# ramkp990/Truth_Recommendation_GNN

Measured on NVIDIA B200. Metric: message-passing edges/s (train step), higher is better.
Workload: dtype f32

## Files before the change

### include/trg_b200.h

```cpp
#ifndef TRG_B200_H
#define TRG_B200_H

#include <stddef.h>
#include <stdint.h>

#ifdef __cplusplus
extern "C" {
#endif

#define TRG_ABI_VERSION 4

enum { TRG_F32 = 0, TRG_BF16 = 1, TRG_F8E4M3 = 2  };
enum {
  TRG_OK = 0,
  TRG_E_ARG = 1,
  TRG_E_WORKSPACE = 2,
  TRG_E_CUDA = 3,
  TRG_E_UNSUPPORTED = 4
};

int trg_abi_version(void);
const char* trg_last_error(void);
int64_t trg_launch_count(void);

size_t trg_csr_workspace_bytes(int64_t n_edges, int64_t n_key);
int trg_csr_build(const int64_t* other, const int64_t* key, int64_t n_edges, int64_t n_key,
                  int32_t* rowptr , int32_t* col , int32_t* eid ,
                  void* workspace, size_t workspace_bytes, void* stream);

size_t trg_select_range_workspace_bytes(int64_t n);
int trg_select_range(const int64_t* key, const int64_t* other, int64_t n, int64_t lo, int64_t hi,
                     int64_t capacity, int64_t pad_key, int64_t pad_other,
                     int64_t* key_out , int64_t* other_out ,
                     int32_t* count_out , void* workspace, size_t workspace_bytes, void* stream);

typedef struct {
  const int32_t* vrowptr;
  const int32_t* vinfo;
  int64_t n_vrows;
  const int32_t* long_rows;
  const int32_t* long_ptr;
  int64_t n_long;
  float* partial;
} trg_long_rows;

int trg_sage_agg_fwd(const int32_t* rowptr, const int32_t* col, const void* x_src,
                     int64_t n_dst, int32_t feat, int dtype,
                     void* mean_out , float* inv_deg_out ,
                     const trg_long_rows* long_rows , void* stream);

int trg_sage_agg_bwd(const int32_t* rowptr_t, const int32_t* col_t, const float* inv_deg,
                     const void* g_mean, int64_t n_src, int32_t feat, int dtype,
                     void* g_src_out , int out_dtype, int accumulate,
                     const void* relu_of, const trg_long_rows* long_rows ,
                     void* stream);

int trg_gather_wsum(const int32_t* rowptr, const int32_t* col, const int32_t* eid,
                    const float* coef, const float* scale, const void* x,
                    int64_t n_rows, int32_t feat, int dtype, void* out, int out_dtype, int accumulate,
                    const void* relu_of, const trg_long_rows* long_rows , void* stream);

int trg_rows_finish(const void* in, int in_dtype, const float* row_scale, const void* add,
                    const void* relu_of, int64_t n_rows, int32_t feat, int dtype, void* out, void* stream);

int trg_peer_reduce_rows(const void* const* parts, int32_t n_peers, int64_t row0, int in_dtype,
                         const float* row_scale, const void* add, const void* relu_of, int64_t n_rows,
                         int32_t feat, int dtype, void* out, int32_t ctas_per_sm, void* stream);

size_t trg_edge_bce_workspace_bytes(int64_t n_users);
int trg_edge_bce_fwd(const int32_t* rowptr_u, const int32_t* col_p, const int32_t* eid,
                     const int64_t* neg_p, const void* u, const void* p,
                     int64_t n_users, int64_t n_edges, int32_t hidden, int dtype,
                     const float* wbar , float* loss_out,
                     float* c_pos, float* c_neg, void* g_u,
                     void* workspace, size_t workspace_bytes, void* stream);

int trg_edge_anchor_loss(const int32_t* rowptr, const int32_t* col, const int32_t* eid,
                         const void* anchor, const void* gathered, int64_t n_rows,
                         int64_t n_edges_scale, int32_t hidden, int dtype, int label,
                         const float* wbar, float* loss_out, float* coef_out, void* g_anchor,
                         int accumulate, int relu_gate, void* workspace, size_t workspace_bytes,
                         void* stream);

typedef struct {
  const void* a;
  const void* w;
  int32_t k;
  float alpha;
} trg_proj_term;
size_t trg_sage_proj_workspace_bytes(int32_t k_total, int32_t hidden, int dtype);
int trg_sage_proj_fwd(const trg_proj_term* terms , int32_t n_terms,
                      const float* bias ,
                      int64_t n_rows, int32_t hidden, int dtype, int relu,
                      void* out ,
                      void* workspace, size_t workspace_bytes, void* stream);

typedef struct {
  const void* w;
  int32_t k;
  float alpha;
  const float* row_scale;
  void* d_a;
} trg_proj_bwd_term;
int trg_sage_proj_bwd_input(const void* dz, const trg_proj_bwd_term* terms , int32_t n_terms,
                            int64_t n_rows, int32_t hidden, int dtype,
                            void* workspace, size_t workspace_bytes, void* stream);

typedef struct {
  const void* a;
  int32_t k;
  float alpha;
  void* d_w;
} trg_proj_dw_term;
size_t trg_sage_proj_dw_workspace_bytes(void);
int trg_sage_proj_bwd_weight(const void* dz, const trg_proj_dw_term* terms , int32_t n_terms,
                             float* d_bias ,
                             int64_t n_rows, int32_t hidden, int dtype,
                             void* workspace, size_t workspace_bytes, void* stream);

size_t trg_score_topk_workspace_bytes(int64_t n_query, int64_t n_cat, int32_t hidden, int32_t k);
int trg_score_topk(const void* q , const void* cat ,
                   int64_t n_query, int64_t n_cat, int32_t hidden, int dtype, int32_t k,
                   int64_t id_offset, float* vals_out , int64_t* ids_out ,
                   void* workspace, size_t workspace_bytes, void* stream);
int trg_score_topk_excluding(const void* q , const void* cat ,
                             int64_t n_query, int64_t n_cat, int32_t hidden, int dtype, int32_t k,
                             int64_t id_offset, const int32_t* excl_rowptr ,
                             const int32_t* excl_ids , const int64_t* query_rows ,
                             float* vals_out , int64_t* ids_out ,
                             void* workspace, size_t workspace_bytes, void* stream);
int trg_topk_merge(const float* vals_in , const int64_t* ids_in,
                   int64_t n_query, int32_t n_lists, int32_t k_in, int32_t k_out,
                   float* vals_out, int64_t* ids_out, void* stream);

size_t trg_rescore_topk_workspace_bytes(int64_t n_query, int32_t n_cand);
int trg_rescore_topk(const void* q , const void* table , int64_t n_query, int64_t n_table,
                     int32_t hidden, int dtype, const int64_t* cand_ids , int32_t n_cand,
                     int64_t id_offset, int32_t k, float* vals_out ,
                     int64_t* ids_out , void* workspace, size_t workspace_bytes, void* stream);

#ifdef __cplusplus
}
#endif
#endif
```

### truth_recommendation_gnn_b200/_lib.py

```python
from __future__ import annotations

import ctypes
import os

import torch

_HERE = os.path.dirname(os.path.abspath(__file__))
LIB_PATH = os.path.join(_HERE, "lib", "libtrg_b200.so")

TRG_F32, TRG_BF16, TRG_F8E4M3 = 0, 1, 2
ABI_VERSION = 4

_vp, _i64, _i32, _sz, _int = ctypes.c_void_p, ctypes.c_int64, ctypes.c_int32, ctypes.c_size_t, ctypes.c_int


class TrgProjTerm(ctypes.Structure):
    _fields_ = [("a", _vp), ("w", _vp), ("k", _i32), ("alpha", ctypes.c_float)]


class TrgLongRows(ctypes.Structure):
    _fields_ = [("vrowptr", _vp), ("vinfo", _vp), ("n_vrows", _i64), ("long_rows", _vp), ("long_ptr", _vp),
                ("n_long", _i64), ("partial", _vp)]


class TrgProjBwdTerm(ctypes.Structure):
    _fields_ = [("w", _vp), ("k", _i32), ("alpha", ctypes.c_float), ("row_scale", _vp), ("d_a", _vp)]


class TrgProjDwTerm(ctypes.Structure):
    _fields_ = [("a", _vp), ("k", _i32), ("alpha", ctypes.c_float), ("d_w", _vp)]


SIGNATURES = {
    "trg_abi_version": (_int, []),
    "trg_last_error": (ctypes.c_char_p, []),
    "trg_launch_count": (_i64, []),
    "trg_csr_workspace_bytes": (_sz, [_i64, _i64]),
    "trg_csr_build": (_int, [_vp, _vp, _i64, _i64, _vp, _vp, _vp, _vp, _sz, _vp]),
    "trg_select_range_workspace_bytes": (_sz, [_i64]),
    "trg_select_range": (_int, [_vp, _vp, _i64, _i64, _i64, _i64, _i64, _i64, _vp, _vp, _vp, _vp, _sz, _vp]),
    "trg_sage_agg_fwd": (_int, [_vp, _vp, _vp, _i64, _i32, _int, _vp, _vp, ctypes.POINTER(TrgLongRows), _vp]),
    "trg_sage_agg_bwd": (_int, [_vp, _vp, _vp, _vp, _i64, _i32, _int, _vp, _int, _int, _vp,
                                ctypes.POINTER(TrgLongRows), _vp]),
    "trg_gather_wsum": (_int, [_vp, _vp, _vp, _vp, _vp, _vp, _i64, _i32, _int, _vp, _int, _int, _vp,
                               ctypes.POINTER(TrgLongRows), _vp]),
    "trg_rows_finish": (_int, [_vp, _int, _vp, _vp, _vp, _i64, _i32, _int, _vp, _vp]),
    "trg_peer_reduce_rows": (_int, [_vp, _i32, _i64, _int, _vp, _vp, _vp, _i64, _i32, _int, _vp, _i32, _vp]),
    "trg_edge_bce_workspace_bytes": (_sz, [_i64]),
    "trg_edge_bce_fwd": (_int, [_vp, _vp, _vp, _vp, _vp, _vp, _i64, _i64, _i32, _int, _vp, _vp,
                                _vp, _vp, _vp, _vp, _sz, _vp]),
    "trg_edge_anchor_loss": (_int, [_vp, _vp, _vp, _vp, _vp, _i64, _i64, _i32, _int, _int, _vp, _vp, _vp,
                                    _vp, _int, _int, _vp, _sz, _vp]),
    "trg_sage_proj_workspace_bytes": (_sz, [_i32, _i32, _int]),
    "trg_sage_proj_fwd": (_int, [ctypes.POINTER(TrgProjTerm), _i32, _vp, _i64, _i32, _int, _int, _vp,
                                 _vp, _sz, _vp]),
    "trg_sage_proj_bwd_input": (_int, [_vp, ctypes.POINTER(TrgProjBwdTerm), _i32, _i64, _i32, _int,
                                       _vp, _sz, _vp]),
    "trg_sage_proj_dw_workspace_bytes": (_sz, []),
    "trg_sage_proj_bwd_weight": (_int, [_vp, ctypes.POINTER(TrgProjDwTerm), _i32, _vp, _i64, _i32, _int,
                                        _vp, _sz, _vp]),
    "trg_score_topk_workspace_bytes": (_sz, [_i64, _i64, _i32, _i32]),
    "trg_score_topk": (_int, [_vp, _vp, _i64, _i64, _i32, _int, _i32, _i64, _vp, _vp, _vp, _sz, _vp]),
    "trg_score_topk_excluding": (_int, [_vp, _vp, _i64, _i64, _i32, _int, _i32, _i64, _vp, _vp, _vp, _vp, _vp,
                                        _vp, _sz, _vp]),
    "trg_topk_merge": (_int, [_vp, _vp, _i64, _i32, _i32, _i32, _vp, _vp, _vp]),
    "trg_rescore_topk_workspace_bytes": (_sz, [_i64, _i32]),
    "trg_rescore_topk": (_int, [_vp, _vp, _i64, _i64, _i32, _int, _vp, _i32, _i64, _i32, _vp, _vp, _vp, _sz,
                                _vp]),
}

_lib = None


class TrgError(RuntimeError):
    pass


def load():
    global _lib
    if _lib is None:
        if not os.path.exists(LIB_PATH):
            raise TrgError(
                f"{LIB_PATH} is missing: build it with `python -m truth_recommendation_gnn_b200.build` "
                "(nvcc, sm_100a). There is no CPU or PyTorch fallback for the hot path.")
        lib = ctypes.CDLL(LIB_PATH)
        for name, (res, args) in SIGNATURES.items():
            fn = getattr(lib, name)
            fn.restype, fn.argtypes = res, args
        if lib.trg_abi_version() != ABI_VERSION:
            raise TrgError("libtrg_b200.so ABI version mismatch; rebuild")
        _lib = lib
    return _lib


def check(rc: int, what: str):
    if rc != 0:
        raise TrgError(f"{what} failed (rc={rc}): {load().trg_last_error().decode()}")


def ptr(t):
    if t is None:
        return None
    if not t.is_cuda:
        raise TrgError("truth_recommendation_gnn_b200 runs on CUDA (sm_100a) tensors only; got a "
                       f"{t.device} tensor. There is no CPU fallback.")
    if not t.is_contiguous():
        raise TrgError("non-contiguous tensor passed to the C ABI")
    return t.data_ptr()


def stream():
    return torch.cuda.current_stream().cuda_stream


def dtype_code(dt: torch.dtype) -> int:
    if dt == torch.float32:
        return TRG_F32
    if dt == torch.bfloat16:
        return TRG_BF16
    raise TrgError(f"unsupported dtype {dt}: the hot path computes in fp32 or bf16 (fp32 accumulate)")


class Profiler:

    def __init__(self):
        self.enabled = False
        self.records = []

    def reset(self):
        self.records = []

    def summary(self):
        out = {}
        for name, nbytes, s, e in self.records:
            d = out.setdefault(name, dict(calls=0, ms=0.0, bytes=0))
            d["calls"] += 1
            d["ms"] += s.elapsed_time(e)
            d["bytes"] += int(nbytes)
        return out


PROF = Profiler()


def call(name, nbytes, fn, *args):
    if PROF.enabled:
        s, e = torch.cuda.Event(enable_timing=True), torch.cuda.Event(enable_timing=True)
        s.record()
        rc = fn(*args)
        e.record()
        PROF.records.append((name, nbytes, s, e))
    else:
        rc = fn(*args)
    check(rc, name)


def launch_count() -> int:
    return int(load().trg_launch_count())
```

### truth_recommendation_gnn_b200/csrc/csr_build.cu

```cuda
#include <algorithm>
#include <cstdio>

#include "common.cuh"

namespace trg {
namespace {

constexpr int kThreads = 256;
constexpr int kItems = 16;
constexpr int kTile = kThreads * kItems;
constexpr int kWarps = kThreads / 32;
constexpr int kRadix = 256;

template <int NWARPS>
__device__ __forceinline__ int block_exclusive_scan(int v, int* warp_sums, int& total) {
  const int lane = threadIdx.x & 31, w = threadIdx.x >> 5;
  int inc = v;
#pragma unroll
  for (int o = 1; o < 32; o <<= 1) {
    int t = __shfl_up_sync(0xffffffffu, inc, o);
    if (lane >= o) inc += t;
  }
  if (lane == 31) warp_sums[w] = inc;
  __syncthreads();
// ... 122 lines not shown
      __trap();
    }
  }
}

__global__ void __launch_bounds__(kThreads)
    select_scatter(const long long* __restrict__ key, const long long* __restrict__ other, int64_t n, long long lo,
                   long long hi, const int* __restrict__ tile_offsets, const int* __restrict__ count,
                   long long capacity, long long pad_key, long long pad_other, long long* __restrict__ key_out,
                   long long* __restrict__ other_out) {
  __shared__ int wtot[kWarps];
  const int lane = threadIdx.x & 31, w = threadIdx.x >> 5;
  const int64_t wbase = (int64_t)blockIdx.x * kTile + (int64_t)w * (kItems * 32);
  long long kv[kItems];
  unsigned sel[kItems];
  int mine = 0;
#pragma unroll
  for (int r = 0; r < kItems; ++r) {
    const int64_t idx = wbase + r * 32 + lane;
    kv[r] = idx < n ? ldg_stream(key + idx) : lo - 1;
    const bool in = kv[r] >= lo && kv[r] < hi;
    sel[r] = __ballot_sync(0xffffffffu, in);
    mine += __popc(sel[r]);
  }
  if (lane == 0) wtot[w] = mine;
  __syncthreads();
  int run = tile_offsets[blockIdx.x];
  for (int i = 0; i < w; ++i) run += wtot[i];
#pragma unroll
  for (int r = 0; r < kItems; ++r) {
    if ((sel[r] >> lane) & 1u) {
      const int dest = run + __popc(sel[r] & ((1u << lane) - 1u));
      if (dest < capacity) {
        key_out[dest] = kv[r] - lo;
        other_out[dest] = ldg_stream(other + wbase + r * 32 + lane);
      }
    }
    run += __popc(sel[r]);
  }
  const long long cnt = *count;
  for (long long i = cnt + (long long)blockIdx.x * kThreads + threadIdx.x; i < capacity;
       i += (long long)gridDim.x * kThreads) {
    key_out[i] = pad_key;
    other_out[i] = pad_other;
  }
}

__device__ __forceinline__ uint2 ldg_pair(const uint2* p) {
  uint2 r;
  asm volatile("ld.global.nc.L1::no_allocate.v2.u32 {%0,%1}, [%2];" : "=r"(r.x), "=r"(r.y) : "l"(p));
  return r;
}
template <bool FIRST>
__device__ __forceinline__ uint32_t load_key(const void* keys, int64_t idx) {
  if (FIRST) return (uint32_t)ldg_stream(reinterpret_cast<const long long*>(keys) + idx);
  return ldg_pair(reinterpret_cast<const uint2*>(keys) + idx).x;
}

template <bool FIRST>
__global__ void __launch_bounds__(kThreads) radix_hist(const void* __restrict__ keys, int64_t n,
                                                       int shift, int* __restrict__ hist,
                                                       int n_ctas) {
  __shared__ int h[kRadix];
  h[threadIdx.x] = 0;
  __syncthreads();
  const int64_t base = (int64_t)blockIdx.x * kTile;
#pragma unroll
  for (int i = 0; i < kItems; ++i) {
    int64_t idx = base + (int64_t)i * kThreads + threadIdx.x;
    if (idx < n) atomicAdd(&h[(load_key<FIRST>(keys, idx) >> shift) & (kRadix - 1)], 1);
  }
  __syncthreads();
  hist[(int64_t)threadIdx.x * n_ctas + blockIdx.x] = h[threadIdx.x];
}

template <bool FIRST, bool LAST>
__global__ void __launch_bounds__(kThreads)
    radix_scatter(const void* __restrict__ keys_in, int64_t n, int shift, const int* __restrict__ gbase,
                  int n_ctas, uint2* __restrict__ pairs_out, uint32_t* __restrict__ vals_out) {
  __shared__ int wcnt[kWarps][kRadix];
  __shared__ int sbase[kRadix];
  const int lane = threadIdx.x & 31, w = threadIdx.x >> 5;
#pragma unroll
  for (int i = 0; i < kWarps; ++i) wcnt[i][threadIdx.x] = 0;
  const int64_t wbase = (int64_t)blockIdx.x * kTile + (int64_t)w * (kItems * 32);

  uint32_t key[kItems], val[kItems];
#pragma unroll
  for (int r = 0; r < kItems; ++r) {
    int64_t idx = wbase + r * 32 + lane;
    bool valid = idx < n;
    if (FIRST) {
      key[r] = valid ? load_key<true>(keys_in, idx) : 0u;
      val[r] = (uint32_t)idx;
    } else {
      const uint2 kv = valid ? ldg_pair(reinterpret_cast<const uint2*>(keys_in) + idx) : make_uint2(0u, 0u);
      key[r] = kv.x;
      val[r] = kv.y;
    }
  }
  __syncthreads();

  int rank[kItems];
#pragma unroll
  for (int r = 0; r < kItems; ++r) {
    const bool valid = wbase + r * 32 + lane < n;
    const int d = valid ? (int)((key[r] >> shift) & (kRadix - 1)) : kRadix;
    const unsigned peers = __match_any_sync(0xffffffffu, d);
    const int prev = valid ? wcnt[w][d] : 0;
    __syncwarp();
    if (valid && lane == __ffs(peers) - 1) wcnt[w][d] = prev + __popc(peers);
    __syncwarp();
    rank[r] = prev + __popc(peers & ((1u << lane) - 1u));
  }
  __syncthreads();
  {
    int run = 0;
#pragma unroll
    for (int i = 0; i < kWarps; ++i) {
      int t = wcnt[i][threadIdx.x];
      wcnt[i][threadIdx.x] = run;
      run += t;
    }
    sbase[threadIdx.x] = gbase[(int64_t)threadIdx.x * n_ctas + blockIdx.x];
  }
  __syncthreads();
#pragma unroll
  for (int r = 0; r < kItems; ++r) {
    if (wbase + r * 32 + lane < n) {
      const int d = (int)((key[r] >> shift) & (kRadix - 1));
      const int dest = sbase[d] + wcnt[w][d] + rank[r];
      if (LAST)
        vals_out[dest] = val[r];
      else
        pairs_out[dest] = make_uint2(key[r], val[r]);
    }
  }
}

__global__ void __launch_bounds__(kThreads) gather_col(const long long* __restrict__ other,
                                                       const int* __restrict__ eid, int64_t n,
                                                       int* __restrict__ col) {
  int64_t i = (int64_t)blockIdx.x * blockDim.x + threadIdx.x;
  const int64_t stride = (int64_t)gridDim.x * blockDim.x;
  for (; i < n; i += stride) col[i] = (int)other[ldg_stream(eid + i)];
}

int num_passes(int64_t n_key) {
  int bits = 1;
  while (bits < 32 && ((int64_t)1 << bits) < n_key) ++bits;
  return (bits + 7) / 8;
}

struct Workspace {
  uint2* pairs[2];
  uint32_t* vals;
  int *hist, *tile_sums;
  size_t bytes;
};

Workspace carve(void* ws, int64_t e, int64_t n_key) {
  Workspace w;
  const size_t ebytes = align_up((size_t)(e > 0 ? e : 1) * 4, 256);
  const int64_t n_ctas = ceil_div<int64_t>(e > 0 ? e : 1, kTile);
  const size_t hist_bytes = align_up((size_t)kRadix * n_ctas * 4, 256);
  const int64_t scan_len = (int64_t)kRadix * n_ctas > n_key + 1 ? (int64_t)kRadix * n_ctas : n_key + 1;
  const size_t sums_bytes = align_up((size_t)ceil_div<int64_t>(scan_len, kTile) * 4 + 4, 256);
  char* p = reinterpret_cast<char*>(ws);
  w.pairs[0] = (uint2*)p; p += 2 * ebytes;
  w.pairs[1] = (uint2*)p; p += 2 * ebytes;
  w.vals = (uint32_t*)p; p += ebytes;
  w.hist = (int*)p; p += hist_bytes;
  w.tile_sums = (int*)p; p += sums_bytes;
  w.bytes = (size_t)(p - reinterpret_cast<char*>(ws));
  return w;
}

}
}

using namespace trg;

extern "C" size_t trg_csr_workspace_bytes(int64_t n_edges, int64_t n_key) {
  if (n_edges < 0 || n_key < 0) return 0;
  return carve(nullptr, n_edges, n_key).bytes;
}

extern "C" int trg_csr_build(const int64_t* other, const int64_t* key, int64_t e, int64_t n_key,
                             int32_t* rowptr, int32_t* col, int32_t* eid, void* workspace,
                             size_t workspace_bytes, void* stream) {
  cudaStream_t st = reinterpret_cast<cudaStream_t>(stream);
  TRG_CHECK_ARG(e >= 0 && n_key >= 0, "trg_csr_build: negative size");
  TRG_CHECK_ARG(e < ((int64_t)1 << 31) && n_key < ((int64_t)1 << 31) - 1,
                "trg_csr_build: n_edges=%lld / n_key=%lld exceed int32 CSR range", (long long)e,
                (long long)n_key);
  TRG_CHECK_ARG(rowptr != nullptr, "trg_csr_build: rowptr is NULL");
  TRG_CHECK_ARG(e == 0 || (key != nullptr && (col == nullptr || other != nullptr)),
                "trg_csr_build: NULL edge arrays with n_edges > 0");
  TRG_CHECK_ARG(e == 0 || n_key > 0, "trg_csr_build: edges present but n_key == 0");
  Workspace w = carve(workspace, e, n_key);
  if (workspace == nullptr || workspace_bytes < w.bytes) {
    set_error("trg_csr_build: workspace %zu < required %zu", workspace_bytes, w.bytes);
    return TRG_E_WORKSPACE;
  }
  TRG_CUDA(cudaMemsetAsync(rowptr, 0, (size_t)(n_key + 1) * sizeof(int32_t), st));
  if (e == 0) return TRG_OK;

  {
    int grid = (int)std::min<int64_t>(ceil_div<int64_t>(e, kThreads), (int64_t)kNumSMs * 16);
    count_keys<<<grid, kThreads, 0, st>>>((const long long*)key, e, (long long)n_key, rowptr);
    count_launch();
    TRG_LAUNCH_OK();
    int rc = exclusive_scan(rowptr, rowptr, n_key + 1, w.tile_sums, st);
    if (rc) return rc;
  }
  if (col == nullptr && eid == nullptr) return TRG_OK;

  const int passes = num_passes(n_key);
  const int n_ctas = (int)ceil_div<int64_t>(e, kTile);
  const void* kin = key;
  const uint32_t* vin = nullptr;
  for (int p = 0; p < passes; ++p) {
    const bool first = p == 0, last = p == passes - 1;
    const int shift = 8 * p;
    uint2* kout = w.pairs[p & 1];
    uint32_t* vout = eid ? (uint32_t*)eid : w.vals;
    if (first)
      radix_hist<true><<<n_ctas, kThreads, 0, st>>>(kin, e, shift, w.hist, n_ctas);
    else
      radix_hist<false><<<n_ctas, kThreads, 0, st>>>(kin, e, shift, w.hist, n_ctas);
    count_launch();
    TRG_LAUNCH_OK();
    int rc = exclusive_scan(w.hist, w.hist, (int64_t)kRadix * n_ctas, w.tile_sums, st);
    if (rc) return rc;
    if (first && last)
      radix_scatter<true, true><<<n_ctas, kThreads, 0, st>>>(kin, e, shift, w.hist, n_ctas, kout, vout);
    else if (first)
      radix_scatter<true, false><<<n_ctas, kThreads, 0, st>>>(kin, e, shift, w.hist, n_ctas, kout, vout);
    else if (last)
      radix_scatter<false, true><<<n_ctas, kThreads, 0, st>>>(kin, e, shift, w.hist, n_ctas, kout, vout);
    else
      radix_scatter<false, false><<<n_ctas, kThreads, 0, st>>>(kin, e, shift, w.hist, n_ctas, kout, vout);
    count_launch();
    TRG_LAUNCH_OK();
    kin = kout;
    vin = vout;
  }
  if (col != nullptr) {
    int grid = (int)std::min<int64_t>(ceil_div<int64_t>(e, kThreads), (int64_t)kNumSMs * 16);
    gather_col<<<grid, kThreads, 0, st>>>((const long long*)other, (const int*)vin, e, col);
    count_launch();
    TRG_LAUNCH_OK();
  }
  return TRG_OK;
}

extern "C" size_t trg_select_range_workspace_bytes(int64_t n) {
  if (n < 0) return 0;
  return align_up((size_t)(ceil_div<int64_t>(n > 0 ? n : 1, kTile) + 1) * 4, 256);
}

extern "C" int trg_select_range(const int64_t* key, const int64_t* other, int64_t n, int64_t lo, int64_t hi,
                                int64_t capacity, int64_t pad_key, int64_t pad_other, int64_t* key_out,
                                int64_t* other_out, int32_t* count_out, void* workspace, size_t workspace_bytes,
                                void* stream) {
  cudaStream_t st = reinterpret_cast<cudaStream_t>(stream);
  TRG_CHECK_ARG(n >= 0 && capacity >= 0 && lo <= hi, "trg_select_range: bad sizes");
  TRG_CHECK_ARG(n < ((int64_t)1 << 31) && capacity < ((int64_t)1 << 31), "trg_select_range: sizes exceed int32 range");
  TRG_CHECK_ARG(count_out && (capacity == 0 || (key_out && other_out)), "trg_select_range: NULL outputs");
  TRG_CHECK_ARG(n == 0 || (key && other), "trg_select_range: NULL inputs with n > 0");
  if (workspace == nullptr || workspace_bytes < trg_select_range_workspace_bytes(n)) {
    set_error("trg_select_range: workspace %zu < required %zu", workspace_bytes, trg_select_range_workspace_bytes(n));
    return TRG_E_WORKSPACE;
  }
  int* tile_counts = reinterpret_cast<int*>(workspace);
  const int n_tiles = (int)ceil_div<int64_t>(n > 0 ? n : 1, kTile);
  select_count<<<n_tiles, kThreads, 0, st>>>((const long long*)key, n, lo, hi, tile_counts);
  select_offsets<<<1, 1024, 0, st>>>(tile_counts, n_tiles, capacity, count_out);
  select_scatter<<<n_tiles, kThreads, 0, st>>>((const long long*)key, (const long long*)other, n, lo, hi, tile_counts,
                                               count_out, capacity, pad_key, pad_other, (long long*)key_out,
                                               (long long*)other_out);
  count_launch(3);
  TRG_LAUNCH_OK();
  return TRG_OK;
}
```

### truth_recommendation_gnn_b200/functional.py

```python
from __future__ import annotations

import ctypes

import torch

from . import _lib, fp8
from .graph import CSR, RelationGraph, build_csr


def _long_rows_arg(csr: CSR, feat: int, dev, elem_size: int = 4):
    lr = csr.long_rows() if feat * elem_size >= 80 else None
    if lr is None:
        return None, None
    partial = torch.empty(lr.n_slots, feat, dtype=torch.float32, device=dev)
    s = _lib.TrgLongRows(_lib.ptr(lr.vrowptr), _lib.ptr(lr.vinfo), int(lr.vinfo.numel()), _lib.ptr(lr.long_rows),
                         _lib.ptr(lr.long_ptr), int(lr.long_rows.numel()), _lib.ptr(partial))
    return ctypes.byref(s), (s, partial)


def _check_rows(x: torch.Tensor, what: str):
    es = x.element_size()
    if x.dim() != 2 or (x.size(1) * es) % 16 != 0:
        raise _lib.TrgError(f"{what}: rows must be a multiple of 16 bytes (got shape {tuple(x.shape)}, "
                            f"{x.dtype}); pad the feature width (the reference pads to 64, inference.py:401-404)")
# ... 29 lines not shown
        raise _lib.TrgError(f"output dtype {out_dtype} is not supported for a {x.dtype} table")
    return out_dtype


def sage_agg_bwd(csr_t: CSR, inv_deg, g_mean: torch.Tensor, out=None, accumulate=False, relu_of=None,
                 out_dtype=None):
    lib = _lib.load()
    g_mean = g_mean.contiguous()
    _check_rows(g_mean, "sage_agg_bwd")
    out_dtype = _out_dtype(g_mean, out, out_dtype)
    _check_epilogue(out, relu_of, csr_t.n_rows, g_mean, "sage_agg_bwd", out_dtype)
    if out is None:
        out = torch.empty(csr_t.n_rows, g_mean.size(1), dtype=out_dtype, device=g_mean.device)
        accumulate = False
    if csr_t.n_rows:
        rb = g_mean.size(1) * g_mean.element_size()
        ob = g_mean.size(1) * out.element_size()
        nbytes = (csr_t.n_edges * (rb + 4) + 4 * (csr_t.n_rows + 1)
                  + csr_t.n_rows * (ob * (1 + bool(accumulate)) + rb * (relu_of is not None))
                  + (4 * csr_t.n_cols if inv_deg is not None else 0))
        lr, keep = _long_rows_arg(csr_t, g_mean.size(1), g_mean.device, g_mean.element_size())
        _lib.call("trg_sage_agg_bwd", nbytes, lib.trg_sage_agg_bwd,
                  _lib.ptr(csr_t.rowptr), _lib.ptr(csr_t.col), _lib.ptr(inv_deg), _lib.ptr(g_mean),
                  csr_t.n_rows, g_mean.size(1), _lib.dtype_code(g_mean.dtype), _lib.ptr(out),
                  _lib.dtype_code(out_dtype), 1 if accumulate else 0, _lib.ptr(relu_of), lr, _lib.stream())
    return out


class SageAggFn(torch.autograd.Function):

    @staticmethod
    def forward(ctx, x_src, rel: RelationGraph, grad_prescaled: bool = False):
        want_inv = rel.inv_deg is None
        mean, inv_deg = sage_agg_fwd(rel.fwd, x_src, want_inv_deg=want_inv)
        if want_inv:
            rel.inv_deg = inv_deg
        ctx.rel = rel
        ctx.grad_prescaled = grad_prescaled
        return mean

    @staticmethod
    def backward(ctx, g_mean):
        if not ctx.needs_input_grad[0]:
            return None, None, None
        rel = ctx.rel
        return sage_agg_bwd(rel.bwd, None if ctx.grad_prescaled else rel.inv_deg, g_mean), None, None


def sage_mean_aggregate(x_src: torch.Tensor, rel: RelationGraph, grad_prescaled: bool = False) -> torch.Tensor:
    return SageAggFn.apply(x_src, rel, grad_prescaled)


def gather_wsum(csr: CSR, coef, x: torch.Tensor, scale=None, out=None, accumulate=False, relu_of=None,
                out_dtype=None):
    lib = _lib.load()
    x = x.contiguous()
    _check_rows(x, "gather_wsum")
    out_dtype = _out_dtype(x, out, out_dtype)
    _check_epilogue(out, relu_of, csr.n_rows, x, "gather_wsum", out_dtype)
    if out is None:
        out = torch.empty(csr.n_rows, x.size(1), dtype=out_dtype, device=x.device)
        accumulate = False
    if csr.n_rows:
        rb = x.size(1) * x.element_size()
        ob = x.size(1) * out.element_size()
        nbytes = (csr.n_edges * (rb + 12) + 4 * (csr.n_rows + 1)
                  + csr.n_rows * (ob * (1 + bool(accumulate)) + rb * (relu_of is not None)))
        lr, keep = _long_rows_arg(csr, x.size(1), x.device, x.element_size())
        _lib.call("trg_gather_wsum", nbytes, lib.trg_gather_wsum,
                  _lib.ptr(csr.rowptr), _lib.ptr(csr.col), _lib.ptr(csr.eid), _lib.ptr(coef),
                  _lib.ptr(scale), _lib.ptr(x), csr.n_rows, x.size(1), _lib.dtype_code(x.dtype),
                  _lib.ptr(out), _lib.dtype_code(out_dtype), 1 if accumulate else 0, _lib.ptr(relu_of), lr,
                  _lib.stream())
    return out


def rows_finish(x, dtype, row_scale=None, add=None, relu_of=None, out=None):
    lib = _lib.load()
    x = x.contiguous()
    n, feat = x.shape
    if x.dtype != dtype and x.dtype != torch.float32:
        raise _lib.TrgError(f"rows_finish: input must be {dtype} or float32, got {x.dtype}")
    for t, what in ((add, "add"), (relu_of, "relu_of"), (out, "out")):
        if t is not None and (t.shape != x.shape or t.dtype != dtype or not t.is_contiguous()):
            raise _lib.TrgError(f"rows_finish: {what} must be a contiguous [{n}, {feat}] {dtype} tensor")
    if out is None:
        out = torch.empty(n, feat, dtype=dtype, device=x.device)
    _check_rows(out, "rows_finish")
    rs = row_scale.float().contiguous() if row_scale is not None else None
    es = out.element_size()
    nbytes = n * feat * (x.element_size() + es * (1 + (add is not None) + (relu_of is not None)))
    _lib.call("trg_rows_finish", nbytes, lib.trg_rows_finish, _lib.ptr(x), _lib.dtype_code(x.dtype), _lib.ptr(rs),
              _lib.ptr(add), _lib.ptr(relu_of), n, feat, _lib.dtype_code(dtype), _lib.ptr(out), _lib.stream())
    return out


def peer_reduce_rows(parts, row0, n_rows, dtype, row_scale=None, add=None, relu_of=None, ctas_per_sm=0):
    import ctypes
    lib = _lib.load()
    feat = parts[0].size(1)
    for t in parts:
        if t.dtype != parts[0].dtype or t.size(1) != feat or t.size(0) < row0 + n_rows or not t.is_contiguous():
            raise _lib.TrgError("peer_reduce_rows: partial tables must be contiguous, of one dtype and width, and "
                                "hold rows [row0, row0 + n_rows)")
    if parts[0].dtype != dtype and parts[0].dtype != torch.float32:
        raise _lib.TrgError(f"peer_reduce_rows: partial tables must be {dtype} or float32")
    for t, what in ((add, "add"), (relu_of, "relu_of")):
        if t is not None and (tuple(t.shape) != (n_rows, feat) or t.dtype != dtype or not t.is_contiguous()):
            raise _lib.TrgError(f"peer_reduce_rows: {what} must be a contiguous [{n_rows}, {feat}] {dtype} tensor")
    out = torch.empty(n_rows, feat, dtype=dtype, device=parts[0].device)
    _check_rows(out, "peer_reduce_rows")
    rs = row_scale.float().contiguous() if row_scale is not None else None
    ptrs = (ctypes.c_void_p * len(parts))(*[_lib.ptr(t) for t in parts])
    nbytes = n_rows * feat * (len(parts) * parts[0].element_size()
                              + out.element_size() * (1 + (add is not None) + (relu_of is not None)))
    _lib.call("trg_peer_reduce_rows", nbytes, lib.trg_peer_reduce_rows, ptrs, len(parts), row0,
              _lib.dtype_code(parts[0].dtype), _lib.ptr(rs), _lib.ptr(add), _lib.ptr(relu_of), n_rows, feat,
              _lib.dtype_code(dtype), _lib.ptr(out), ctas_per_sm, _lib.stream())
    return out


class LinkStructure:

    def __init__(self, train_edge_index, interaction_type_tensor, num_users, num_posts):
        pos_u, pos_p = train_edge_index[0], train_edge_index[1]
        self.train_edge_index = train_edge_index
        self.num_users, self.num_posts = int(num_users), int(num_posts)
        self.n_edges = int(pos_u.numel())
        self.by_user = build_csr(pos_p, pos_u, self.num_users, self.num_posts)
        self.by_post = build_csr(pos_u, pos_p, self.num_posts, self.num_users, validate=False)
        self._by_post_u = None
        self._user_of_u = None
        if self.n_edges:
            w = interaction_type_tensor[pos_p + num_users].float()
            self.wbar = w.mean().reshape(1).contiguous()
        else:
            self.wbar = torch.full((1,), float("nan"), device=pos_u.device)


    @property
    def by_post_u(self) -> CSR:
        if self._by_post_u is None:
            bu, bp = self.by_user, self.by_post
            inv = torch.empty(self.n_edges, dtype=torch.int32, device=bu.eid.device)
            inv[bu.eid.long()] = torch.arange(self.n_edges, dtype=torch.int32, device=bu.eid.device)
            self._by_post_u = CSR(bp.rowptr, bp.col, inv[bp.eid.long()].contiguous(), bp.n_rows, bp.n_cols, bp._long)
        return self._by_post_u

    @property
    def user_of_u(self) -> torch.Tensor:
        if self._user_of_u is None:
            rp = self.by_user.rowptr.long()
            self._user_of_u = torch.repeat_interleave(
                torch.arange(self.num_users, device=rp.device), rp[1:] - rp[:-1]).contiguous()
        return self._user_of_u


_LINK_CACHE: dict = {}


def link_structure(train_edge_index, interaction_type_tensor, num_users, num_posts) -> LinkStructure:
    key = (train_edge_index.data_ptr(), tuple(train_edge_index.shape), train_edge_index._version,
           interaction_type_tensor.data_ptr(), interaction_type_tensor._version, int(num_users),
           int(num_posts))
    s = _LINK_CACHE.get(key)
    if s is None:
        if len(_LINK_CACHE) > 8:
            _LINK_CACHE.clear()
        s = LinkStructure(train_edge_index, interaction_type_tensor, num_users, num_posts)
        s._keepalive = interaction_type_tensor
        _LINK_CACHE[key] = s
    return s


def edge_bce_fwd(ls: LinkStructure, user_emb, post_emb, neg_p, want_grad: bool):
    lib = _lib.load()
    _check_rows(user_emb, "edge_bce_fwd")
    if user_emb.dtype != post_emb.dtype or user_emb.size(1) != post_emb.size(1):
        raise _lib.TrgError("user and post embeddings must share dtype and width")
    if neg_p.dtype != torch.int64 or neg_p.numel() != ls.n_edges:
        raise _lib.TrgError("neg_p must be int64 with one entry per positive edge (train_gnn.py:272)")
    user_emb, post_emb, neg_p = user_emb.contiguous(), post_emb.contiguous(), neg_p.contiguous()
    dev = user_emb.device
    loss = torch.empty(1, dtype=torch.float32, device=dev)
    c_pos = c_neg = g_u = None
    if want_grad:
        c_pos = torch.empty(ls.n_edges, dtype=torch.float32, device=dev)
        c_neg = torch.empty(ls.n_edges, dtype=torch.float32, device=dev)
        g_u = torch.empty_like(user_emb)
    ws_bytes = int(lib.trg_edge_bce_workspace_bytes(ls.num_users))
    ws = torch.empty(ws_bytes, dtype=torch.uint8, device=dev)
    e = ls.n_edges
    e_scale = int(getattr(ls, "n_edges_scale", e))
    rb = user_emb.size(1) * user_emb.element_size()
    nbytes = e * (2 * rb + 16 + (8 if want_grad else 0)) + ls.num_users * (rb * (2 if want_grad else 1) + 4)
    _lib.call("trg_edge_bce_fwd", nbytes, lib.trg_edge_bce_fwd,
              _lib.ptr(ls.by_user.rowptr), _lib.ptr(ls.by_user.col) if e else None,
              _lib.ptr(ls.by_user.eid) if e else None, _lib.ptr(neg_p) if e else None,
              _lib.ptr(user_emb), _lib.ptr(post_emb), ls.num_users, e_scale, user_emb.size(1),
              _lib.dtype_code(user_emb.dtype), _lib.ptr(ls.wbar), _lib.ptr(loss), _lib.ptr(c_pos),
              _lib.ptr(c_neg), _lib.ptr(g_u), _lib.ptr(ws), ws_bytes, _lib.stream())
    return loss, c_pos, c_neg, g_u


def edge_anchor_loss(csr: CSR, anchor, gathered, n_edges_scale, label, wbar, want_grad, g_anchor=None,
                     relu_gate=False, coef_in_csr_order=False):
    lib = _lib.load()
    anchor, gathered = anchor.contiguous(), gathered.contiguous()
    _check_rows(anchor, "edge_anchor_loss")
    dev = anchor.device
    loss = torch.empty(1, dtype=torch.float32, device=dev)
    coef = None
    accumulate = g_anchor is not None
    if want_grad:
        coef = torch.empty(csr.n_edges, dtype=torch.float32, device=dev)
        if g_anchor is None:
            g_anchor = torch.empty_like(anchor)
    else:
        g_anchor = None
    ws_bytes = int(lib.trg_edge_bce_workspace_bytes(csr.n_rows))
    ws = torch.empty(ws_bytes, dtype=torch.uint8, device=dev)
    e = csr.n_edges
    rb = anchor.size(1) * anchor.element_size()
    nbytes = e * (rb + 12) + csr.n_rows * (rb * (2 if want_grad else 1) + 4)
    _lib.call("trg_edge_anchor_loss", nbytes, lib.trg_edge_anchor_loss,
              _lib.ptr(csr.rowptr), _lib.ptr(csr.col) if e else None,
              _lib.ptr(csr.eid) if (e and not coef_in_csr_order) else None,
              _lib.ptr(anchor), _lib.ptr(gathered), csr.n_rows, int(n_edges_scale), anchor.size(1),
              _lib.dtype_code(anchor.dtype), 1 if label else 0, _lib.ptr(wbar), _lib.ptr(loss), _lib.ptr(coef),
              _lib.ptr(g_anchor), 1 if (accumulate and want_grad) else 0,
              1 if (relu_gate and want_grad) else 0, _lib.ptr(ws), ws_bytes, _lib.stream())
    return loss, coef, g_anchor


class LinkBCEFn(torch.autograd.Function):

    @staticmethod
    def forward(ctx, user_emb, post_emb, neg_p, ls: LinkStructure):
        want = user_emb.requires_grad or post_emb.requires_grad
        if neg_p.dtype != torch.int64 or neg_p.numel() != ls.n_edges:
            raise _lib.TrgError("neg_p must be int64 with one entry per positive edge (train_gnn.py:272)")
        if getattr(ls, "eid_long", None) is None:
            ls.eid_long = ls.by_user.eid.long()
        e_scale = int(getattr(ls, "n_edges_scale", ls.n_edges))
        bu = ls.by_user
        ctx.neg_by_post = None
        if want and ls.n_edges:
            ctx.neg_by_post = build_csr(ls.train_edge_index[0], neg_p, ls.num_posts, ls.num_users, validate=False,
                                        per_step=True)
        col_neg = neg_p.index_select(0, ls.eid_long).int()
        neg_csr = CSR(bu.rowptr, col_neg, bu.eid, bu.n_rows, bu.n_cols)
        l_pos, c_pos, g_u = edge_anchor_loss(bu, user_emb, post_emb, e_scale, 1, ls.wbar, want, None)
        l_neg, c_neg, g_u = edge_anchor_loss(neg_csr, user_emb, post_emb, e_scale, 0, ls.wbar, want, g_u)
        ctx.ls = ls
        ctx.want = want
        if want:
            ctx.save_for_backward(user_emb, neg_p, c_pos, c_neg, g_u)
        return (l_pos + l_neg).reshape(())

    @staticmethod
    def backward(ctx, g):
        user_emb, neg_p, c_pos, c_neg, g_u = ctx.saved_tensors
        ls = ctx.ls
        g = g.reshape(1).float().contiguous()
        g_user = g_post = None
        if ctx.needs_input_grad[0]:
            g_user = g_u * g.to(g_u.dtype)
        if ctx.needs_input_grad[1]:
            g_post = gather_wsum(ls.by_post, c_pos, user_emb, scale=g)
            if ctx.neg_by_post is not None:
                gather_wsum(ctx.neg_by_post, c_neg, user_emb, scale=g, out=g_post, accumulate=True)
        return g_user, g_post, None, None


def link_bce_loss(user_emb, post_emb, train_edge_index, neg_p, interaction_type_tensor, num_users):
    ls = link_structure(train_edge_index, interaction_type_tensor, num_users, post_emb.size(0))
    return LinkBCEFn.apply(user_emb, post_emb, neg_p, ls)


def _proj_bytes(n, ks, hidden, es):
    return n * (sum(ks) + hidden) * es


def sage_proj_fwd(terms, bias, relu: bool):
    lib = _lib.load()
    a0 = terms[0][0]
    n, hidden = a0.size(0), terms[0][1].size(0)
    arr = (_lib.TrgProjTerm * len(terms))()
    keep = []
    for i, (a, w, alpha) in enumerate(terms):
        a, w = a.contiguous(), w.contiguous()
        if a.dtype != a0.dtype or w.dtype != a0.dtype:
            raise _lib.TrgError("projection operands must share one dtype")
        keep += [a, w]
        arr[i].a, arr[i].w, arr[i].k, arr[i].alpha = _lib.ptr(a), _lib.ptr(w), a.size(1), float(alpha)
    out = torch.empty(n, hidden, dtype=a0.dtype, device=a0.device)
    b = bias.float().contiguous() if bias is not None else None
    ktot = sum(t[0].size(1) for t in terms)
    code = _lib.dtype_code(a0.dtype)
    ws_bytes = int(lib.trg_sage_proj_workspace_bytes(ktot, hidden, code))
    ws = torch.empty(ws_bytes, dtype=torch.uint8, device=a0.device)
    _lib.call("trg_sage_proj_fwd", _proj_bytes(n, [t[0].size(1) for t in terms], hidden, a0.element_size()),
              lib.trg_sage_proj_fwd, arr, len(terms), _lib.ptr(b), n, hidden, code, 1 if relu else 0,
              _lib.ptr(out), _lib.ptr(ws), ws_bytes, _lib.stream())
    return out


def sage_proj_bwd_input(dz, terms):
    lib = _lib.load()
    dz = dz.contiguous()
    n, hidden = dz.shape
    arr = (_lib.TrgProjBwdTerm * len(terms))()
    outs, keep = [], []
    for i, (w, alpha, rs) in enumerate(terms):
        w = w.contiguous()
        if w.dtype != dz.dtype:
            raise _lib.TrgError("projection operands must share one dtype")
        d_a = torch.empty(n, w.size(1), dtype=dz.dtype, device=dz.device)
        rs = rs.float().contiguous() if rs is not None else None
        keep += [w, rs]
        outs.append(d_a)
        arr[i].w, arr[i].k, arr[i].alpha = _lib.ptr(w), w.size(1), float(alpha)
        arr[i].row_scale, arr[i].d_a = _lib.ptr(rs), _lib.ptr(d_a)
    ktot = sum(t[0].size(1) for t in terms)
    code = _lib.dtype_code(dz.dtype)
# ... 133 lines not shown
```

### truth_recommendation_gnn_b200/fused_step.py

```python
from __future__ import annotations

import torch

from . import _lib
from .functional import (edge_anchor_loss, gather_wsum, link_structure, sage_agg_bwd, sage_agg_fwd,
                         sage_proj_bwd_input, sage_proj_bwd_weight, sage_proj_fwd)
from .graph import CSR, build_csr, relation_graph
from .nn import REL_DIRECT, REL_ENGAGE, REL_SOCIAL, StackedWeightedRGCN, WeightedRGCN


def _layers(model):
    if type(model) is StackedWeightedRGCN:
        return list(model.layers)
    if type(model) is WeightedRGCN:
        return [model]
    return None


def model_eligible(model) -> bool:
    layers = _layers(model)
    if layers is None or not torch.is_grad_enabled():
        return False
    if any(conv.lin_l.bias is None for l in layers for conv in (l.msg_direct, l.msg_social, l.post_update)):
        return False
    return all(p.requires_grad for p in model.parameters())


def eligible(model, x_dict) -> bool:
    if not model_eligible(model):
        return False
    xu, xp = x_dict["user"], x_dict["post"]
    return xu.is_cuda and xp.is_cuda and not xu.requires_grad and not xp.requires_grad and xu.dtype == xp.dtype


def _agg(rel, x):
    want_inv = rel.inv_deg is None
    mean, inv_deg = sage_agg_fwd(rel.fwd, x, want_inv_deg=want_inv)
    if want_inv:
        rel.inv_deg = inv_deg
    return mean


@torch.no_grad()
def loss_and_grads(model, x_dict, edge_index_dict, train_edge_index, interaction_type_tensor, num_users,
                   neg_p, neg_ready=None):
    layers = _layers(model)
    if layers is None:
        raise _lib.TrgError("loss_and_grads: model must be WeightedRGCN or StackedWeightedRGCN")
    hu, hp = x_dict["user"].contiguous(), x_dict["post"].contiguous()
    n_u, n_p = hu.size(0), hp.size(0)
    rel_d = relation_graph(edge_index_dict[REL_DIRECT], n_p, n_u)
    rel_s = relation_graph(edge_index_dict[REL_SOCIAL], n_u, n_u)
    rel_e = relation_graph(edge_index_dict[REL_ENGAGE], n_u, n_p)

    saved = []
    for layer in layers:
        layer.materialize(hu.size(-1), hp.size(-1))
        mean_d, mean_s, mean_e = _agg(rel_d, hp), _agg(rel_s, hu), _agg(rel_e, hu)
        ug, pg = layer.user_gemm(), layer.post_gemm()
        hu_n = sage_proj_fwd(ug.terms(mean_d, mean_s, hu), ug.bias, True)
        hp_n = sage_proj_fwd(pg.terms(mean_e, hp), pg.bias, True)
        saved.append((hu, hp, mean_d, mean_s, mean_e, ug, pg))
        hu, hp = hu_n, hp_n

    ls = link_structure(train_edge_index, interaction_type_tensor, num_users, n_p)
    if neg_ready is not None:
        torch.cuda.current_stream().wait_event(neg_ready)
    if neg_p.dtype != torch.int64 or neg_p.numel() != ls.n_edges:
        raise _lib.TrgError("neg_p must be int64 with one entry per positive edge (train_gnn.py:272)")
    if getattr(ls, "eid_long", None) is None:
        ls.eid_long = ls.by_user.eid.long()
    bu = ls.by_user
    col_neg64 = neg_p.index_select(0, ls.eid_long)
    neg_by_post = build_csr(ls.user_of_u, col_neg64, n_p, n_u, validate=False, per_step=True)
    neg_by_user = CSR(bu.rowptr, col_neg64.int(), bu.eid, bu.n_rows, bu.n_cols)
    l_pos, c_pos, dz_u = edge_anchor_loss(bu, hu, hp, ls.n_edges, 1, ls.wbar, True, None, coef_in_csr_order=True)
    l_neg, c_neg, dz_u = edge_anchor_loss(neg_by_user, hu, hp, ls.n_edges, 0, ls.wbar, True, dz_u,
                                          relu_gate=True, coef_in_csr_order=True)
    dz_p = gather_wsum(ls.by_post_u, c_pos, hu)
    gather_wsum(neg_by_post, c_neg, hu, out=dz_p, accumulate=True, relu_of=hp)
    del col_neg64
    loss = (l_pos + l_neg).reshape(())
    del neg_by_user, neg_by_post, c_pos, c_neg, hu, hp

    for li in range(len(layers) - 1, -1, -1):
        hu_in, hp_in, mean_d, mean_s, mean_e, ug, pg = saved.pop()
        dw_u, db_u = sage_proj_bwd_weight(dz_u, ug.dw_terms(mean_d, mean_s, hu_in), True)
        dw_p, db_p = sage_proj_bwd_weight(dz_p, pg.dw_terms(mean_e, hp_in), True)
        del mean_d, mean_s, mean_e
        layers[li].accumulate_grads(dw_u, db_u, dw_p, db_p)
        if li == 0:
            break
        g_md, g_ms, g_hu = sage_proj_bwd_input(dz_u, ug.dx_terms(rel_d.inv_deg, rel_s.inv_deg, None))
        g_me, g_hp = sage_proj_bwd_input(dz_p, pg.dx_terms(rel_e.inv_deg, None))
        del dz_u, dz_p
        sage_agg_bwd(rel_s.bwd, None, g_ms, out=g_hu, accumulate=True)
        sage_agg_bwd(rel_e.bwd, None, g_me, out=g_hu, accumulate=True, relu_of=hu_in)
        sage_agg_bwd(rel_d.bwd, None, g_md, out=g_hp, accumulate=True, relu_of=hp_in)
        dz_u, dz_p = g_hu, g_hp
    return loss
```

Baseline: 2.968 billion.

## Fuse per-step negative gather and CSR build into dedicated radix kernel

Replaces the per-step index_select of negatives, int64-to-int32 conversion and generic build_csr with a custom trg_group_negatives routine. A single front kernel gathers the negatives in by-user order, writes the int32 column, counts post degrees and builds the first radix histogram. The radix scatter is then staged through shared memory and carries the user id along, so eid and col are written directly on the last pass. This removes several PyTorch launches and int64 intermediates from each train step, at the cost of more custom code and an ABI bump.

Result: faster. 3.008 billion, median of 6 (+1.3%).

```diff
diff --git a/include/trg_b200.h b/include/trg_b200.h
--- a/include/trg_b200.h
+++ b/include/trg_b200.h
@@ -8,7 +8,7 @@
 extern "C" {
 #endif
 
-#define TRG_ABI_VERSION 4
+#define TRG_ABI_VERSION 5
 
 enum { TRG_F32 = 0, TRG_BF16 = 1, TRG_F8E4M3 = 2  };
 enum {
@@ -27,6 +27,12 @@
 int trg_csr_build(const int64_t* other, const int64_t* key, int64_t n_edges, int64_t n_key,
                   int32_t* rowptr , int32_t* col , int32_t* eid ,
                   void* workspace, size_t workspace_bytes, void* stream);
+
+size_t trg_group_negatives_workspace_bytes(int64_t n_edges, int64_t n_key);
+int trg_group_negatives(const int64_t* neg , const int32_t* eid_by_user ,
+                        const int32_t* user_of_pos , int64_t n_edges, int64_t n_key,
+                        int32_t* col_by_user , int32_t* rowptr , int32_t* col ,
+                        int32_t* eid , void* workspace, size_t workspace_bytes, void* stream);
 
 size_t trg_select_range_workspace_bytes(int64_t n);
 int trg_select_range(const int64_t* key, const int64_t* other, int64_t n, int64_t lo, int64_t hi,
diff --git a/truth_recommendation_gnn_b200/_lib.py b/truth_recommendation_gnn_b200/_lib.py
--- a/truth_recommendation_gnn_b200/_lib.py
+++ b/truth_recommendation_gnn_b200/_lib.py
@@ -9,7 +9,7 @@
 LIB_PATH = os.path.join(_HERE, "lib", "libtrg_b200.so")
 
 TRG_F32, TRG_BF16, TRG_F8E4M3 = 0, 1, 2
-ABI_VERSION = 4
+ABI_VERSION = 5
 
 _vp, _i64, _i32, _sz, _int = ctypes.c_void_p, ctypes.c_int64, ctypes.c_int32, ctypes.c_size_t, ctypes.c_int
 
@@ -37,6 +37,8 @@
     "trg_launch_count": (_i64, []),
     "trg_csr_workspace_bytes": (_sz, [_i64, _i64]),
     "trg_csr_build": (_int, [_vp, _vp, _i64, _i64, _vp, _vp, _vp, _vp, _sz, _vp]),
+    "trg_group_negatives_workspace_bytes": (_sz, [_i64, _i64]),
+    "trg_group_negatives": (_int, [_vp, _vp, _vp, _i64, _i64, _vp, _vp, _vp, _vp, _vp, _sz, _vp]),
     "trg_select_range_workspace_bytes": (_sz, [_i64]),
     "trg_select_range": (_int, [_vp, _vp, _i64, _i64, _i64, _i64, _i64, _i64, _vp, _vp, _vp, _vp, _sz, _vp]),
     "trg_sage_agg_fwd": (_int, [_vp, _vp, _vp, _i64, _i32, _int, _vp, _vp, ctypes.POINTER(TrgLongRows), _vp]),
diff --git a/truth_recommendation_gnn_b200/csrc/csr_build.cu b/truth_recommendation_gnn_b200/csrc/csr_build.cu
--- a/truth_recommendation_gnn_b200/csrc/csr_build.cu
+++ b/truth_recommendation_gnn_b200/csrc/csr_build.cu
@@ -298,14 +298,164 @@
   return (bits + 7) / 8;
 }
 
+__global__ void __launch_bounds__(kThreads)
+    negatives_front(const long long* __restrict__ neg, const int* __restrict__ eid, int64_t n, long long n_key,
+                    int* __restrict__ col_by_user, int* __restrict__ deg, int* __restrict__ hist, int n_ctas) {
+  __shared__ int h[kRadix];
+  h[threadIdx.x] = 0;
+  __syncthreads();
+  const int64_t base = (int64_t)blockIdx.x * kTile + threadIdx.x;
+  int e[kItems];
+#pragma unroll
+  for (int i = 0; i < kItems; ++i) {
+    const int64_t idx = base + (int64_t)i * kThreads;
+    e[i] = idx < n ? ldg_stream(eid + idx) : -1;
+  }
+  long long k[kItems];
+#pragma unroll
+  for (int i = 0; i < kItems; ++i) k[i] = e[i] >= 0 ? __ldg(neg + e[i]) : 0;
+#pragma unroll
+  for (int i = 0; i < kItems; ++i) {
+    const int64_t idx = base + (int64_t)i * kThreads;
+    if (idx < n) {
+      if ((unsigned long long)k[i] >= (unsigned long long)n_key) {
+        printf("trg_group_negatives: negative %lld at by-user position %lld is outside [0, %lld)\n", k[i],
+               (long long)idx, n_key);
+        __trap();
+      }
+      col_by_user[idx] = (int)k[i];
+      atomicAdd(&deg[(int)k[i]], 1);
+      atomicAdd(&h[(int)k[i] & (kRadix - 1)], 1);
+    }
+  }
+  __syncthreads();
+  hist[(int64_t)threadIdx.x * n_ctas + blockIdx.x] = h[threadIdx.x];
+}
+
+constexpr int kStagedSmem = kTile * (int)(sizeof(uint2) + sizeof(uint32_t));
+template <bool FIRST, bool LAST>
+__global__ void __launch_bounds__(kThreads, 3)
+    radix_scatter_staged(const void* __restrict__ keys_in, const uint32_t* __restrict__ users_in, int64_t n,
+                         int shift, const int* __restrict__ gbase, int n_ctas, uint2* __restrict__ pairs_out,
+                         uint32_t* __restrict__ users_out, int* __restrict__ eid_out, int* __restrict__ col_out) {
+  __shared__ int wcnt[kWarps][kRadix];
+  __shared__ int sloc[kRadix];
+  __shared__ int sdest[kRadix];
+  __shared__ int warp_sums[kWarps];
+  extern __shared__ uint2 stage[];
+  uint32_t* stage_user = reinterpret_cast<uint32_t*>(stage + kTile);
+  const int lane = threadIdx.x & 31, w = threadIdx.x >> 5;
+#pragma unroll
+  for (int i = 0; i < kWarps; ++i) wcnt[i][threadIdx.x] = 0;
+  const int64_t tbase = (int64_t)blockIdx.x * kTile;
+  const int64_t wbase = tbase + (int64_t)w * (kItems * 32);
+  const int gb = gbase[(int64_t)threadIdx.x * n_ctas + blockIdx.x];
+
+  uint32_t key[kItems], val[kItems];
+#pragma unroll
+  for (int r = 0; r < kItems; ++r) {
+    const int64_t idx = wbase + r * 32 + lane;
+    const bool valid = idx < n;
+    if (FIRST) {
+      key[r] = valid ? (uint32_t)ldg_stream(reinterpret_cast<const int*>(keys_in) + idx) : 0u;
+      val[r] = (uint32_t)idx;
+    } else {
+      const uint2 kv = valid ? ldg_pair(reinterpret_cast<const uint2*>(keys_in) + idx) : make_uint2(0u, 0u);
+      key[r] = kv.x;
+      val[r] = kv.y;
+    }
+  }
+  __syncthreads();
+
+  int rank[kItems];
+#pragma unroll
+  for (int r = 0; r < kItems; ++r) {
+    const bool valid = wbase + r * 32 + lane < n;
+    const int d = valid ? (int)((key[r] >> shift) & (kRadix - 1)) : kRadix;
+    const unsigned peers = __match_any_sync(0xffffffffu, d);
+    const int prev = valid ? wcnt[w][d] : 0;
+    __syncwarp();
+    if (valid && lane == __ffs(peers) - 1) wcnt[w][d] = prev + __popc(peers);
+    __syncwarp();
+    rank[r] = prev + __popc(peers & ((1u << lane) - 1u));
+  }
+  __syncthreads();
+  {
+    int run = 0;
+#pragma unroll
+    for (int i = 0; i < kWarps; ++i) {
+      const int t = wcnt[i][threadIdx.x];
+      wcnt[i][threadIdx.x] = run;
+      run += t;
+    }
+    int total;
+    const int loc = block_exclusive_scan<kWarps>(run, warp_sums, total);
+    sloc[threadIdx.x] = loc;
+    sdest[threadIdx.x] = gb - loc;
+  }
+  __syncthreads();
+#pragma unroll
+  for (int r = 0; r < kItems; ++r) {
+    if (wbase + r * 32 + lane < n) {
+      const int d = (int)((key[r] >> shift) & (kRadix - 1));
+      rank[r] += sloc[d] + wcnt[w][d];
+      stage[rank[r]] = make_uint2(key[r], val[r]);
+    }
+  }
+  {
+    uint32_t user[kItems];
+#pragma unroll
+    for (int r = 0; r < kItems; ++r) {
+      const int64_t idx = wbase + r * 32 + lane;
+      user[r] = idx < n ? (uint32_t)ldg_stream(reinterpret_cast<const int*>(users_in) + idx) : 0u;
+    }
+#pragma unroll
+    for (int r = 0; r < kItems; ++r)
+      if (wbase + r * 32 + lane < n) stage_user[rank[r]] = user[r];
+  }
+  __syncthreads();
+  const int cnt = (int)(n - tbase < kTile ? n - tbase : kTile);
+  uint2 kv[kItems];
+#pragma unroll
+  for (int r = 0; r < kItems; ++r) {
+    const int p = r * kThreads + threadIdx.x;
+    kv[r] = p < cnt ? stage[p] : make_uint2(0u, 0u);
+  }
+#pragma unroll
+  for (int r = 0; r < kItems; ++r) {
+    const int p = r * kThreads + threadIdx.x;
+    if (p < cnt) {
+      const int dest = sdest[(kv[r].x >> shift) & (kRadix - 1)] + p;
+      if (LAST) {
+        eid_out[dest] = (int)kv[r].y;
+        col_out[dest] = (int)stage_user[p];
+      } else {
+        pairs_out[dest] = kv[r];
+        users_out[dest] = stage_user[p];
+      }
+    }
+  }
+}
+
+template <bool FIRST, bool LAST>
+int launch_staged(const void* keys_in, const uint32_t* users_in, int64_t n, int shift, const int* gbase, int n_ctas,
+                  uint2* pairs_out, uint32_t* users_out, int* eid_out, int* col_out, cudaStream_t st) {
+  static SmemAttrState attr;
+  TRG_CUDA(ensure_dyn_smem(radix_scatter_staged<FIRST, LAST>, kStagedSmem, attr));
+  radix_scatter_staged<FIRST, LAST><<<n_ctas, kThreads, kStagedSmem, st>>>(keys_in, users_in, n, shift, gbase, n_ctas,
+                                                                           pairs_out, users_out, eid_out, col_out);
+  return TRG_OK;
+}
+
 struct Workspace {
   uint2* pairs[2];
   uint32_t* vals;
+  uint32_t* users[2];
   int *hist, *tile_sums;
   size_t bytes;
 };
 
-Workspace carve(void* ws, int64_t e, int64_t n_key) {
+Workspace carve(void* ws, int64_t e, int64_t n_key, bool negatives = false) {
   Workspace w;
   const size_t ebytes = align_up((size_t)(e > 0 ? e : 1) * 4, 256);
   const int64_t n_ctas = ceil_div<int64_t>(e > 0 ? e : 1, kTile);
@@ -315,7 +465,13 @@
   char* p = reinterpret_cast<char*>(ws);
   w.pairs[0] = (uint2*)p; p += 2 * ebytes;
   w.pairs[1] = (uint2*)p; p += 2 * ebytes;
-  w.vals = (uint32_t*)p; p += ebytes;
+  w.vals = w.users[0] = w.users[1] = nullptr;
+  if (negatives) {
+    w.users[0] = (uint32_t*)p; p += ebytes;
+    w.users[1] = (uint32_t*)p; p += ebytes;
+  } else {
+    w.vals = (uint32_t*)p; p += ebytes;
+  }
   w.hist = (int*)p; p += hist_bytes;
   w.tile_sums = (int*)p; p += sums_bytes;
   w.bytes = (size_t)(p - reinterpret_cast<char*>(ws));
@@ -401,6 +557,71 @@
   return TRG_OK;
 }
 
+extern "C" size_t trg_group_negatives_workspace_bytes(int64_t n_edges, int64_t n_key) {
+  if (n_edges < 0 || n_key < 0) return 0;
+  return carve(nullptr, n_edges, n_key, true).bytes;
+}
+
+extern "C" int trg_group_negatives(const int64_t* neg, const int32_t* eid_by_user, const int32_t* user_of_pos,
+                                   int64_t e, int64_t n_key, int32_t* col_by_user, int32_t* rowptr, int32_t* col,
+                                   int32_t* eid, void* workspace, size_t workspace_bytes, void* stream) {
+  cudaStream_t st = reinterpret_cast<cudaStream_t>(stream);
+  TRG_CHECK_ARG(e >= 0 && n_key >= 0, "trg_group_negatives: negative size");
+  TRG_CHECK_ARG(e < ((int64_t)1 << 31) && n_key < ((int64_t)1 << 31) - 1,
+                "trg_group_negatives: n_edges=%lld / n_key=%lld exceed int32 CSR range", (long long)e,
+                (long long)n_key);
+  TRG_CHECK_ARG(rowptr != nullptr, "trg_group_negatives: rowptr is NULL");
+  TRG_CHECK_ARG(e == 0 || (neg && eid_by_user && user_of_pos && col_by_user && col && eid),
+                "trg_group_negatives: NULL edge arrays with n_edges > 0");
+  TRG_CHECK_ARG(e == 0 || n_key > 0, "trg_group_negatives: edges present but n_key == 0");
+  Workspace w = carve(workspace, e, n_key, true);
+  if (workspace == nullptr || workspace_bytes < w.bytes) {
+    set_error("trg_group_negatives: workspace %zu < required %zu", workspace_bytes, w.bytes);
+    return TRG_E_WORKSPACE;
+  }
+  TRG_CUDA(cudaMemsetAsync(rowptr, 0, (size_t)(n_key + 1) * sizeof(int32_t), st));
+  if (e == 0) return TRG_OK;
+
+  const int n_ctas = (int)ceil_div<int64_t>(e, kTile);
+  negatives_front<<<n_ctas, kThreads, 0, st>>>((const long long*)neg, eid_by_user, e, (long long)n_key,
+                                               col_by_user, rowptr, w.hist, n_ctas);
+  count_launch();
+  TRG_LAUNCH_OK();
+  int rc = exclusive_scan(rowptr, rowptr, n_key + 1, w.tile_sums, st);
+  if (rc) return rc;
+
+  const int passes = num_passes(n_key);
+  const void* kin = col_by_user;
+  for (int p = 0; p < passes; ++p) {
+    const bool first = p == 0, last = p == passes - 1;
+    const int shift = 8 * p;
+    uint2* kout = w.pairs[p & 1];
+    if (!first) {
+      radix_hist<false><<<n_ctas, kThreads, 0, st>>>(kin, e, shift, w.hist, n_ctas);
+      count_launch();
+      TRG_LAUNCH_OK();
+    }
+    rc = exclusive_scan(w.hist, w.hist, (int64_t)kRadix * n_ctas, w.tile_sums, st);
+    if (rc) return rc;
+    const uint32_t* uin = first ? (const uint32_t*)user_of_pos : w.users[(p + 1) & 1];
+    uint32_t* uout = w.users[p & 1];
+    int rc2;
+    if (first && last)
+      rc2 = launch_staged<true, true>(kin, uin, e, shift, w.hist, n_ctas, kout, uout, eid, col, st);
+    else if (first)
+      rc2 = launch_staged<true, false>(kin, uin, e, shift, w.hist, n_ctas, kout, uout, eid, col, st);
+    else if (last)
+      rc2 = launch_staged<false, true>(kin, uin, e, shift, w.hist, n_ctas, kout, uout, eid, col, st);
+    else
+      rc2 = launch_staged<false, false>(kin, uin, e, shift, w.hist, n_ctas, kout, uout, eid, col, st);
+    if (rc2) return rc2;
+    count_launch();
+    TRG_LAUNCH_OK();
+    kin = kout;
+  }
+  return TRG_OK;
+}
+
 extern "C" size_t trg_select_range_workspace_bytes(int64_t n) {
   if (n < 0) return 0;
   return align_up((size_t)(ceil_div<int64_t>(n > 0 ? n : 1, kTile) + 1) * 4, 256);
diff --git a/truth_recommendation_gnn_b200/functional.py b/truth_recommendation_gnn_b200/functional.py
--- a/truth_recommendation_gnn_b200/functional.py
+++ b/truth_recommendation_gnn_b200/functional.py
@@ -205,7 +205,7 @@
         if self._user_of_u is None:
             rp = self.by_user.rowptr.long()
             self._user_of_u = torch.repeat_interleave(
-                torch.arange(self.num_users, device=rp.device), rp[1:] - rp[:-1]).contiguous()
+                torch.arange(self.num_users, dtype=torch.int32, device=rp.device), rp[1:] - rp[:-1]).contiguous()
         return self._user_of_u
 
 
@@ -224,6 +224,30 @@
         s._keepalive = interaction_type_tensor
         _LINK_CACHE[key] = s
     return s
+
+
+def group_negatives(ls: LinkStructure, neg_p):
+    lib = _lib.load()
+    if neg_p.dtype != torch.int64 or neg_p.numel() != ls.n_edges:
+        raise _lib.TrgError("neg_p must be int64 with one entry per positive edge (train_gnn.py:272)")
+    neg_p = neg_p.contiguous()
+    bu, e, n_p = ls.by_user, ls.n_edges, ls.num_posts
+    dev = bu.rowptr.device
+    user_of_u = ls.user_of_u if e else None
+    col_by_user = torch.empty(e, dtype=torch.int32, device=dev)
+    rowptr = torch.empty(n_p + 1, dtype=torch.int32, device=dev)
+    col = torch.empty(e, dtype=torch.int32, device=dev)
+    eid = torch.empty(e, dtype=torch.int32, device=dev)
+    ws_bytes = int(lib.trg_group_negatives_workspace_bytes(e, n_p))
+    ws = torch.empty(ws_bytes, dtype=torch.uint8, device=dev)
+    nbytes = e * 28 + 8 * (n_p + 1)
+    _lib.call("trg_group_negatives", nbytes, lib.trg_group_negatives,
+              _lib.ptr(neg_p) if e else None, _lib.ptr(bu.eid) if e else None, _lib.ptr(user_of_u), e, n_p,
+              _lib.ptr(col_by_user) if e else None, _lib.ptr(rowptr), _lib.ptr(col) if e else None,
+              _lib.ptr(eid) if e else None, _lib.ptr(ws), ws_bytes, _lib.stream())
+    neg_by_user = CSR(bu.rowptr, col_by_user, bu.eid, bu.n_rows, bu.n_cols)
+    neg_by_post = CSR(rowptr, col, eid, n_p, ls.num_users, False)
+    return neg_by_user, neg_by_post
 
 
 def edge_bce_fwd(ls: LinkStructure, user_emb, post_emb, neg_p, want_grad: bool):
diff --git a/truth_recommendation_gnn_b200/fused_step.py b/truth_recommendation_gnn_b200/fused_step.py
--- a/truth_recommendation_gnn_b200/fused_step.py
+++ b/truth_recommendation_gnn_b200/fused_step.py
@@ -3,9 +3,9 @@
 import torch
 
 from . import _lib
-from .functional import (edge_anchor_loss, gather_wsum, link_structure, sage_agg_bwd, sage_agg_fwd,
-                         sage_proj_bwd_input, sage_proj_bwd_weight, sage_proj_fwd)
-from .graph import CSR, build_csr, relation_graph
+from .functional import (edge_anchor_loss, gather_wsum, group_negatives, link_structure, sage_agg_bwd,
+                         sage_agg_fwd, sage_proj_bwd_input, sage_proj_bwd_weight, sage_proj_fwd)
+from .graph import relation_graph
 from .nn import REL_DIRECT, REL_ENGAGE, REL_SOCIAL, StackedWeightedRGCN, WeightedRGCN
 
 
@@ -66,20 +66,13 @@
     ls = link_structure(train_edge_index, interaction_type_tensor, num_users, n_p)
     if neg_ready is not None:
         torch.cuda.current_stream().wait_event(neg_ready)
-    if neg_p.dtype != torch.int64 or neg_p.numel() != ls.n_edges:
-        raise _lib.TrgError("neg_p must be int64 with one entry per positive edge (train_gnn.py:272)")
-    if getattr(ls, "eid_long", None) is None:
-        ls.eid_long = ls.by_user.eid.long()
     bu = ls.by_user
-    col_neg64 = neg_p.index_select(0, ls.eid_long)
-    neg_by_post = build_csr(ls.user_of_u, col_neg64, n_p, n_u, validate=False, per_step=True)
-    neg_by_user = CSR(bu.rowptr, col_neg64.int(), bu.eid, bu.n_rows, bu.n_cols)
+    neg_by_user, neg_by_post = group_negatives(ls, neg_p)
     l_pos, c_pos, dz_u = edge_anchor_loss(bu, hu, hp, ls.n_edges, 1, ls.wbar, True, None, coef_in_csr_order=True)
     l_neg, c_neg, dz_u = edge_anchor_loss(neg_by_user, hu, hp, ls.n_edges, 0, ls.wbar, True, dz_u,
                                           relu_gate=True, coef_in_csr_order=True)
     dz_p = gather_wsum(ls.by_post_u, c_pos, hu)
     gather_wsum(neg_by_post, c_neg, hu, out=dz_p, accumulate=True, relu_of=hp)
-    del col_neg64
     loss = (l_pos + l_neg).reshape(())
     del neg_by_user, neg_by_post, c_pos, c_neg, hu, hp
 
```
